# ZhengkunTian/OpenTransformer

Hardware: AMD Instinct MI355X
Metric: utterances/sec (80-d fbank, ~1000 frames) train fwd+bwd (higher is better)
Workload: dtype fp16; 1 GPU; AISHELL-1 transformer_baseline.yaml (+input_size 80), 12 enc / 6 dec layers, B=32/GPU x 1000 frames x 80-d fbank, 15 decoder rows, V=4234, residual_dropout 0.1; step = fwd + bwd + grad all-reduce + clip/Adam/Noam; global_batch=32, frames=1000, parallelism=dp1, hipgraph=True

## Files before the change

include/otrans_hip.h:

```cpp
#ifndef OTRANS_HIP_H
#define OTRANS_HIP_H
#include <stddef.h>
#include <stdint.h>
#ifdef __cplusplus
extern "C" {
#endif

#define OTR_F32 0
#define OTR_BF16 1
#define OTR_F16 2
#define OTR_ACT_NONE 0
#define OTR_ACT_RELU 1

#define OTR_ABI_VERSION 604
int32_t otr_version(void);
int32_t otr_half_type(void);
int32_t otr_debug_set(int32_t key, int32_t value);
int32_t otr_set_fault_counter(void* device_word);
int32_t otr_debug_trread(const void* image, const int32_t* addr, void* out, void* stream);
int32_t otr_debug_trace(void* buf);
const char* otr_last_error_string(void);

typedef struct {
  int32_t M, N, K;
// ... 178 lines not shown
  int32_t act_dtype, compute;
  int32_t w_dtype;
} otr_conv_desc_t;
int32_t otr_conv1_fwd(const otr_conv_desc_t* d, const float* x, const float* w1, const float* b1, void* act1,
                      void* stream);
int32_t otr_conv1_wgrad(const otr_conv_desc_t* d, const float* x, const void* dact1, float* dw1, float* db1,
                        float* partial, void* stream);
int32_t otr_conv1_wgrad_partial_rows(void);
int32_t otr_conv2_fwd(const otr_conv_desc_t* d, const void* act1, const void* w2r, const float* b2, void* act2,
                      void* stream);
int32_t otr_conv12_fwd(const otr_conv_desc_t* d, const float* x, const float* w1, const float* b1, void* act1, const void* w2r,
                       const float* b2, void* act2, void* stream);
int32_t otr_conv2_dgrad_cols(const otr_conv_desc_t* d, const void* dact2, const void* w2r, void* dcol,
                             void* stream);
int32_t otr_conv2_col2im(const otr_conv_desc_t* d, const void* dcol, const void* act1, void* dact1, void* stream);
int32_t otr_conv2_dgrad(const otr_conv_desc_t* d, const void* dact2, const void* w2r, const void* act1, void* dact1,
                        void* stream);
int64_t otr_conv2_wide_scratch_bytes(void);
int32_t otr_conv2_dgrad_wide(const otr_conv_desc_t* d, const void* dact2, const void* w2r, const void* act1, void* dact1, void* scratch,
                             int64_t scratch_bytes, void* stream);
int32_t otr_debug_conv2_dgrad_plan(const otr_conv_desc_t* d, int32_t* out);
int32_t otr_conv2_wgrad(const otr_conv_desc_t* d, const void* dact2, const void* act1, float* dw2r, void* workspace,
                        int64_t workspace_bytes, void* stream);
int32_t otr_relu_bwd(const void* y, const void* g, void* out, int32_t dtype, int64_t n, void* stream);
int32_t otr_relu_bwd_colsum_partial_rows(int64_t rows, int32_t cols, int32_t dtype);
int32_t otr_relu_bwd_colsum(const void* y, const void* g, void* out, float* partial, int32_t dtype, int64_t rows, int32_t cols,
                            void* stream);

int32_t otr_act_fwd(const void* x, void* y, int32_t dtype, int64_t n, int32_t kind, void* stream);
int32_t otr_act_bwd(const void* x, const void* dy, void* dx, int32_t dtype, int64_t n, int32_t kind, void* stream);

int32_t otr_label_smoothing_loss(const float* logits, const int64_t* target, int64_t R, int32_t V, float smoothing,
                                 int32_t pad_idx, float* loss, float* dlogits, float* scratch, void* stream);
int32_t otr_label_smoothing_loss_ld(const float* logits, int64_t ld_logits, const int64_t* target, int64_t R, int32_t V,
                                    float smoothing, int32_t pad_idx, float* loss, float* dlogits, int64_t ld_dlogits,
                                    float* scratch, void* stream);

int32_t otr_label_smoothing_loss_fused(const float* logits, int64_t ld_logits, const int64_t* target, int64_t ld_target, int32_t L,
                                       int64_t R, int32_t V, float smoothing, int32_t pad_idx, const float* grad_scale, float* loss,
                                       void* dlogits, int32_t dlogits_dtype, int64_t ld_dlogits, float* scratch, uint32_t* ticket,
                                       void* stream);

int32_t otr_log_softmax(const float* x, float* y, int64_t R, int32_t V, void* stream);

int32_t otr_residual_add_fwd(const float* x, const void* a, int32_t a_dtype, float* y, int64_t n, float scale,
                             float p_drop, const uint64_t* seed, uint64_t rng_offset, void* stream);
// ... 197 lines not shown
```

opentransformer_amd/_lib.py:

```python
import ctypes as C
import os

_HERE = os.path.dirname(os.path.abspath(__file__))
_LIB_DIR = os.environ.get('OTR_LIB_DIR') or os.path.join(_HERE, 'lib')
LIB_PATHS = {'bf16': os.path.join(_LIB_DIR, 'libotrans_hip.so'), 'fp16': os.path.join(_LIB_DIR, 'libotrans_hip_f16.so')}
LIB_PATH = LIB_PATHS['bf16']

OTR_F32, OTR_BF16, OTR_F16 = 0, 1, 2
OTR_ABI_VERSION = 604
OTR_OPT_STATE_FLOATS = 528
ACT_NONE, ACT_RELU = 0, 1


class LinearDesc(C.Structure):
    _fields_ = [('M', C.c_int32), ('N', C.c_int32), ('K', C.c_int32),
                ('x_dtype', C.c_int32), ('w_dtype', C.c_int32), ('y_dtype', C.c_int32), ('compute', C.c_int32),
                ('ldx', C.c_int64), ('ldw', C.c_int64), ('ldy', C.c_int64),
                ('act', C.c_int32), ('accumulate', C.c_int32)]


class WgradItem(C.Structure):
    _fields_ = [('dy', C.c_void_p), ('x', C.c_void_p), ('dw', C.c_void_p), ('M', C.c_int32), ('N', C.c_int32),
                ('K', C.c_int32), ('ldy', C.c_int64), ('ldx', C.c_int64), ('ldw', C.c_int64),
                ('dy_dtype', C.c_int32), ('x_dtype', C.c_int32), ('dbias', C.c_void_p), ('overwrite', C.c_int32)]
# ... 109 lines not shown
    'otr_glu_fwd': [_P, _P, _I32, _I64, _I64, _P, _P],
    'otr_glu_bwd': [_P, _P, _P, _P, _I32, _I64, _I64, _P, _I32, _P],
    'otr_posenc_fwd': [_P, _P, _P, _I64, _I32, _I32, _F32, _P],
    'otr_posenc_mask_fwd': [_P, _P, _P, _I64, _I32, _I32, _F32, _P, _I64, _I64, _P, _P],
    'otr_embed_posenc_fwd': [_P, _P, _P, _P, _I64, _I32, _I32, _I32, _F32, _P],
    'otr_embed_posenc_fwd_ld': [_P, _I64, _P, _P, _P, _I64, _I32, _I32, _I32, _F32, _P],
    'otr_embed_bwd_ld': [_P, _I64, _I32, _P, _P, _I32, _P, _I64, _I32, _I32, _F32, _P],
    'otr_embed_bwd': [_P, _P, _P, _I64, _I32, _I32, _F32, _P],
    'otr_scale': [_P, _P, _I64, _P, _F32, _P],
    'otr_scale_cast': [_P, _P, _I64, _F32, _P],
    'otr_cast_f32_to_bf16': [_P, _P, _I64, _P],
    'otr_conv1_fwd': [C.POINTER(ConvDesc), _P, _P, _P, _P, _P],
    'otr_conv1_wgrad': [C.POINTER(ConvDesc), _P, _P, _P, _P, _P, _P],
    'otr_conv1_wgrad_partial_rows': [],
    'otr_conv2_fwd': [C.POINTER(ConvDesc), _P, _P, _P, _P, _P],
    'otr_conv12_fwd': [C.POINTER(ConvDesc), _P, _P, _P, _P, _P, _P, _P, _P],
    'otr_conv2_dgrad_cols': [C.POINTER(ConvDesc), _P, _P, _P, _P],
    'otr_conv2_col2im': [C.POINTER(ConvDesc), _P, _P, _P, _P],
    'otr_conv2_dgrad': [C.POINTER(ConvDesc), _P, _P, _P, _P, _P],
    'otr_conv2_wide_scratch_bytes': [],
    'otr_conv2_dgrad_wide': [C.POINTER(ConvDesc), _P, _P, _P, _P, _P, _I64, _P],
    'otr_debug_conv2_dgrad_plan': [C.POINTER(ConvDesc), _P],
    'otr_conv2_wgrad': [C.POINTER(ConvDesc), _P, _P, _P, _P, _I64, _P],
    'otr_relu_bwd': [_P, _P, _P, _I32, _I64, _P],
    'otr_relu_bwd_colsum_partial_rows': [_I64, _I32, _I32],
    'otr_relu_bwd_colsum': [_P, _P, _P, _P, _I32, _I64, _I32, _P],
    'otr_act_fwd': [_P, _P, _I32, _I64, _I32, _P],
    'otr_act_bwd': [_P, _P, _P, _I32, _I64, _I32, _P],
    'otr_label_smoothing_loss': [_P, _P, _I64, _I32, _F32, _I32, _P, _P, _P, _P],
    'otr_label_smoothing_loss_ld': [_P, _I64, _P, _I64, _I32, _F32, _I32, _P, _P, _I64, _P, _P],
    'otr_label_smoothing_loss_fused': [_P, _I64, _P, _I64, _I32, _I64, _I32, _F32, _I32, _P, _P, _P, _I32, _I64, _P, _P, _P],
    'otr_log_softmax': [_P, _P, _I64, _I32, _P],
    'otr_ctc_loss': [_P, _P, _I64, _P, _P, _I32, _I32, _I32, _I32, _I32, _P, _P, _P, _P, _P],
    'otr_ffn_fwd_split_slab': [_P, _P, _P, _P, _P, _P, _P, _I64, _I32, _I32, _P],
    'otr_ffn_bwd_split_slab': [_P, _P, _P, _P, _P, _P, _I64, _I32, _I32, _P],
    'otr_ln_bwd_proj_slabs': [_P, _P, _I32, _P, _P, _P, _P, _P, _P, _P, _P, _P, _I64, _P, _I64, _I32, _F32, C.c_uint64, _P],
    'otr_rb_linear_ln': [C.POINTER(DecLn), _P, _P, _P, _I32, _I64, _I64, _I32, _I32, _P],
    'otr_dec_self_fwd': [C.POINTER(DecLn), _I32, _I32, _P, _P, _P, _P, _P, _P, _P, _P],
    'otr_dec_self_step': [C.POINTER(DecLn), _I64, _P, _P, _P, _P, _P, _P, _P, _I32, _P, _P],
    'otr_dec_cross_fwd': [C.POINTER(DecLn), _I32, _I32, _P, _P, _P, _P, _I64, _I64, _I32, _I32, _P, _I32, _P, _P, _P, _P, _P],
    'otr_dec_cross_fwd_shared': [C.POINTER(DecLn), _I32, _I32, _P, _P, _P, _P, _I64, _I64, _I32, _I32, _P, _I32, _I32, _P, _P, _P, _P, _P],
    'otr_dec_ffn_hsave_bytes': [_I64, _I32],
    'otr_dec_ffn_fwd': [C.POINTER(DecLn), _I64, _P, _P, _P, _I32, _I32, _P, _P, _P],
    'otr_dec_ln': [C.POINTER(DecLn), _I64, _P],
    'otr_dec_self_step_pair': [C.POINTER(DecSelfStep), C.POINTER(DecSelfStep), _P],
    'otr_dec_ffn_fwd_pair': [C.POINTER(DecFfnFwd), C.POINTER(DecFfnFwd), _P],
# ... 116 lines not shown
```

opentransformer_amd/csrc/api.hip:

```cpp
#include <stdarg.h>
#include <stdio.h>
#include <stdlib.h>

#include <algorithm>
#include <vector>

#include "gemm_kernel.h"
#include "wgrad256.h"

static thread_local char g_err[512] = "";

void otr_set_error(const char* fmt, ...) {
  va_list ap;
  va_start(ap, fmt);
  vsnprintf(g_err, sizeof(g_err), fmt, ap);
  va_end(ap);
}

int32_t otr_check_launch(const char* what) {
  hipError_t e = hipGetLastError();
  if (e != hipSuccess) {
    otr_set_error("%s: launch failed: %s", what, hipGetErrorString(e));
    return (int32_t)e;
  }
// ... 369 lines not shown
}

extern "C" int32_t otr_conv2_dgrad_cols(const otr_conv_desc_t* d, const void* dact2, const void* w2r, void* dcol,
                                        void* stream) {
  GemmArgs a{};
  if (int32_t e = conv_geom(d, a.cg)) return e;
  OTR_REQUIRE(dact2 && w2r && dcol, "conv2_dgrad_cols: null pointer");
  a.A = dact2; a.B = w2r; a.C = dcol; a.bias = nullptr;
  a.M = d->B * d->T2 * d->F2; a.N = 9 * d->C1; a.K = d->C2;
  a.lda = d->C2; a.ldb = 9 * d->C1; a.ldc = 9 * d->C1;
  a.act = OTR_ACT_NONE; a.accumulate = 0;
  a.a_vec = kc_vec(dact2, a.lda, d->act_dtype);
  OTR_REQUIRE(dtype_ok(d->w_dtype), "conv2_dgrad_cols: bad w_dtype");
  a.b_vec = mc_vec(w2r, a.ldb, d->w_dtype, d->compute);
  return run_gemm(a, d->compute, d->act_dtype, d->w_dtype, d->act_dtype, MODE_KC, MODE_MC, stream);
}

extern "C" int32_t otr_conv2_wgrad(const otr_conv_desc_t* d, const void* dact2, const void* act1, float* dw2r,
                                   void* workspace, int64_t workspace_bytes, void* stream) {
  GemmArgs a{};
  if (int32_t e = conv_geom(d, a.cg)) return e;
  OTR_REQUIRE(dact2 && act1 && dw2r, "conv2_wgrad: null pointer");
  if (g_otr_conv2_wgrad256 && d->act_dtype == OTR_H16 && d->compute == OTR_H16) {
    const int32_t rc = wgrad256_conv_launch(dact2, act1, dw2r, d->B, d->T1, d->F1, d->T2, d->F2, d->C1, d->C2, workspace, workspace_bytes,
                                            (hipStream_t)stream);
    if (rc != 1) return rc;
  }
  a.A = dact2; a.B = act1; a.C = dw2r; a.bias = nullptr;
  a.M = d->C2; a.N = 9 * d->C1; a.K = d->B * d->T2 * d->F2;
  a.lda = d->C2; a.ldb = 0; a.ldc = 9 * d->C1;
  a.act = OTR_ACT_NONE; a.accumulate = 0;
  a.a_vec = mc_vec(dact2, a.lda, d->act_dtype, d->compute);
  a.b_vec = ((uintptr_t)act1 % 16 == 0);
  a.allow_split = 1; a.ws = (float*)workspace; a.ws_bytes = workspace_bytes; a.trace = g_otr_trace;
  return run_gemm(a, d->compute, d->act_dtype, d->act_dtype, OTR_F32, MODE_MC, MODE_IM2M, stream);
}
```

opentransformer_amd/csrc/wgrad256.h:

```cpp
#pragma once
#include <hip/hip_runtime.h>
#include <stdint.h>

#include "common.h"

constexpr int W256_MAX_PROBS = 56;

struct W256Item {
  const void* dy;
  const void* x;
  float* dw;
  float* dbias;
  int M, N, K;
  int64_t ldy, ldx, ldw;
  int overwrite;
};

struct W256Prob {
  const uint16_t* dy;
  const uint16_t* x;
  float* dw;
  float* dbias;
  int start;
  int M, N, K, ldy, ldx, ldw;
  int flag0;
};

struct W256Args {
  W256Prob p[W256_MAX_PROBS];
  int total, chunk;
  int mode, nfull, rem_tiles, parts;
  int nprob, spin_limit;
  int cT1, cF1, cT2, cF2, cC1;
  FastDiv cdivF2, cdivT2;
  float* split_ws;
  int* flags;
  const void* zeros;
  int* fault;
};

int32_t wgrad256_launch(const W256Item* items, int n, void* workspace, int64_t workspace_bytes, int grid_cap, hipStream_t s);
int64_t wgrad256_workspace_bytes(const W256Item* items, int n);
int32_t wgrad256_conv_launch(const void* g2, const void* act1, float* dw2r, int B, int T1, int F1, int T2, int F2, int C1, int C2,
                             void* workspace, int64_t workspace_bytes, hipStream_t s);
```

opentransformer_amd/csrc/wgrad256.hip:

```cpp
#include "common.h"
#include "wgrad256.h"

#include <algorithm>

namespace {

typedef short v4s __attribute__((ext_vector_type(4)));
typedef __attribute__((address_space(3))) v4s lds_v4s;

constexpr int SLAB_ROWS = 16;
constexpr int SLAB_BYTES = 16384;
constexpr int RING = 8, AHEAD = 6;
constexpr int LDS_BYTES = RING * SLAB_BYTES;

__device__ __forceinline__ uint2 tr_read(uint32_t lds_addr) {
  v4s r = __builtin_amdgcn_ds_read_tr16_b64_v4i16((lds_v4s*)(uintptr_t)lds_addr);
  return __builtin_bit_cast(uint2, r);
}

struct Frags {
  uint4 a[4], b[2];
};

__device__ __forceinline__ void read_frags_lo(Frags& f, uint32_t slab_addr, uint32_t a_off, uint32_t b_off) {
// ... 24 lines not shown
#else
  typedef __bf16 hv2 __attribute__((ext_vector_type(2)));
  const hv2 one = {(__bf16)1.f, (__bf16)1.f};
#define W256_DOT(w, c) __builtin_amdgcn_fdot2_f32_bf16(__builtin_bit_cast(hv2, w), one, c, false)
#endif
#pragma unroll
  for (int a = 0; a < 4; ++a) {
    cs[a] = W256_DOT(f.a[a].x, cs[a]);
    cs[a] = W256_DOT(f.a[a].y, cs[a]);
    cs[a] = W256_DOT(f.a[a].z, cs[a]);
    cs[a] = W256_DOT(f.a[a].w, cs[a]);
  }
#undef W256_DOT
}

struct Stager {
  const unsigned char* base_a;
  const unsigned char* base_b;
  int64_t step_a, step_b;
  int row0, M;
  bool col_a, col_b;
  const unsigned char* zeros;
  uint32_t dst;
  int cT1, cF1, cT2, cF2, kh, kw;
  int64_t pix_bytes;
  FastDiv divF2, divT2;
  template <bool NTA, bool NTB, bool CONV = false> __device__ __forceinline__ void issue(int slab, int slot) {
    const bool ok = slab * SLAB_ROWS + row0 < M;
    const unsigned char* pa = ok && col_a ? base_a + slab * step_a : zeros;
    const unsigned char* pb;
    if constexpr (CONV) {
      const uint32_t m = (uint32_t)(slab * SLAB_ROWS + row0);
      const uint32_t t = fdiv(m, divF2), f2 = m - t * (uint32_t)cF2, b = fdiv(t, divT2), t2 = t - b * (uint32_t)cT2;
      const int fin = 2 * (int)f2 + kw - 1;
      const bool in = ok && col_b && fin >= 0 && fin < cF1;
      pb = in ? base_b + (((int64_t)b * cT1 + 2 * (int)t2 + kh) * cF1 + fin) * pix_bytes : zeros;
    } else {
      pb = ok && col_b ? base_b + slab * step_b : zeros;
    }
    lds_dma<NTA>(pa, (uint32_t)(slot * SLAB_BYTES) + dst);
    lds_dma<NTB>(pb, (uint32_t)(slot * SLAB_BYTES) + 8192u + dst);
  }
};

template <bool NTA, bool NTB, bool BIAS, bool CONV = false>
__device__ __forceinline__ void stream_piece(Stager& sg, f32x16 (&acc)[4][2], float (&cs)[4], int wc, int sb, int P, int rot,
                                             uint32_t a_off, uint32_t b_off) {
  int stage = rot;
  auto issue_next = [&](int slot) {
    sg.issue<NTA, NTB, CONV>(sb + stage, slot);
    stage = stage + 1 == P ? 0 : stage + 1;
  };
#pragma unroll
  for (int j = 0; j < AHEAD; ++j)
    if (j < P) issue_next(j);
  if (P >= AHEAD) wait_vm<2 * (AHEAD - 2)>(); else wait_vm<0>();
  __builtin_amdgcn_s_barrier();
  __builtin_amdgcn_sched_barrier(0);
  asm volatile("" ::: "memory");
  Frags f0, f1;
  read_frags_lo(f0, 0u, a_off, b_off);
  read_frags_hi(f0, 0u, a_off, b_off);
#define W256_MMA(A, CUR)                                                                                     \
  mma32(acc[A][0], CUR.a[A], CUR.b[0]);                                                                      \
  mma32(acc[A][1], CUR.a[A], CUR.b[1]);                                                                      \
  __builtin_amdgcn_sched_barrier(0);
#define W256_PHASE(Q, CUR, NXT, ST)                                                                          \
  {                                                                                                          \
    const int q_ = (Q);                                                                                      \
    const bool more_ = (ST) || q_ + AHEAD < P, next_ = (ST) || q_ + 1 < P;                      \
    const uint32_t nslab_ = (uint32_t)(((q_ + 1) & (RING - 1)) * SLAB_BYTES);                                \
    W256_MMA(0, CUR)                                                                                         \
    if (more_) issue_next((q_ + AHEAD) & (RING - 1));                                                        \
    __builtin_amdgcn_sched_barrier(0);                                                                       \
    W256_MMA(1, CUR)                                                                                         \
    if (next_) read_frags_lo(NXT, nslab_, a_off, b_off);                                                     \
    __builtin_amdgcn_sched_barrier(0);                                                                       \
    W256_MMA(2, CUR)                                                                                         \
    if (next_) read_frags_hi(NXT, nslab_, a_off, b_off);                                                     \
    __builtin_amdgcn_sched_barrier(0);                                                                       \
    W256_MMA(3, CUR)                                                                                         \
    if constexpr (BIAS) { if ((q_ & 3) == wc) frag_colsum(cs, CUR); }     \
    if (more_) wait_vm<2 * (AHEAD - 2)>(); else wait_vm<0>();                                                \
    __builtin_amdgcn_s_barrier();                                                                            \
    asm volatile("" ::: "memory");                                                                           \
    __builtin_amdgcn_sched_barrier(0);                                                                       \
  }
  int q = 0;
  for (; q + AHEAD + 1 < P; q += 2) {
    W256_PHASE(q, f0, f1, true)
    W256_PHASE(q + 1, f1, f0, true)
  }
  for (; q + 1 < P; q += 2) {
    W256_PHASE(q, f0, f1, false)
    W256_PHASE(q + 1, f1, f0, false)
  }
  if (q < P) W256_PHASE(q, f0, f1, false)
#undef W256_PHASE
#undef W256_MMA
}

template <bool COH, bool FIRST = false>
__device__ __forceinline__ void flush_tile(f32x16 (&acc)[4][2], float* dw, int ldw, int N, int K, int n_base, int k_base,
                                           unsigned char* scr, int lane) {
  constexpr int AUX = COH ? 17 : 0;
  const int rr = lane >> 3, cq = lane & 7;
// ... 40 lines not shown
  }
}

template <bool COH> __device__ __forceinline__ void flush_bias(const float (&cs)[4], float* dbias, int N, int n_base, int lane) {
  constexpr int AUX = COH ? 17 : 0;
  auto rs = __builtin_amdgcn_make_buffer_rsrc(dbias, 0, N * 4, 0x00020000);
#pragma unroll
  for (int a = 0; a < 4; ++a) {
    const uint32_t off = (uint32_t)((n_base + 32 * a + lane) * 4);
    const float old = __uint_as_float(__builtin_amdgcn_raw_buffer_load_b32(rs, off, 0, AUX));
    __builtin_amdgcn_raw_buffer_store_b32(__float_as_uint(old + cs[a]), rs, off, 0, AUX);
  }
}

__global__ void trread_probe_kernel(const uint16_t* image, const int* addr, uint16_t* out) {
  __shared__ __attribute__((aligned(16))) uint16_t img[2048];
  for (int i = threadIdx.x; i < 2048; i += 64) img[i] = image[i];
  __syncthreads();
  const uint2 r = tr_read((uint32_t)(uintptr_t)(lds_byte*)reinterpret_cast<unsigned char*>(img) + (uint32_t)addr[threadIdx.x]);
  out[threadIdx.x * 4 + 0] = (uint16_t)(r.x & 0xffffu); out[threadIdx.x * 4 + 1] = (uint16_t)(r.x >> 16);
  out[threadIdx.x * 4 + 2] = (uint16_t)(r.y & 0xffffu); out[threadIdx.x * 4 + 3] = (uint16_t)(r.y >> 16);
}

__global__ void wgrad256_init_kernel(int* flags, int n, uint32_t* zeros) {
  for (int i = threadIdx.x; i < n; i += blockDim.x) flags[i] = 0;
  if (threadIdx.x < 16) zeros[threadIdx.x] = 0u;
}

template <bool CONV = false>
__global__ __launch_bounds__(512) void wgrad256_kernel(W256Args g) {
  __shared__ __attribute__((aligned(1024))) unsigned char smem[LDS_BYTES];
  const int tid = threadIdx.x, lane = tid & 63;
  const int wid = __builtin_amdgcn_readfirstlane(tid >> 6);
  const int wr = wid >> 2, wc = wid & 3;
  const uint32_t smem0 = (uint32_t)(uintptr_t)(lds_byte*)smem;

  const int gq = lane >> 4, p16 = lane & 15;
  const uint32_t lane_off = (uint32_t)((4 * (gq >> 1) + (p16 >> 2)) * 64 + (gq & 1) * 32 + (p16 & 3) * 8);
  const uint32_t a_off = smem0 + lane_off + (uint32_t)(4 * wr) * 512u;
  const uint32_t b_off = smem0 + lane_off + 8192u + (uint32_t)(2 * wc) * 512u;

  const int st_row = 8 * (wid >> 2) + ((lane >> 2) & 7);
  const int st_col = 64 * (wid & 3) + 32 * (lane >> 5) + 8 * (lane & 3);

  const int G = (int)gridDim.x, gx = G >> 3, bid = (int)blockIdx.x;
  const bool rounds = g.mode >= 1;
  const int slot = (G & 7) == 0 ? (bid & 7) * gx + (rounds ? (bid >> 3) : gx - 1 - (bid >> 3)) : (rounds ? bid : G - 1 - bid);
  int pos = slot * g.chunk;
  const int c_end = pos + g.chunk < g.total ? pos + g.chunk : g.total;
  int round = 0;

  for (;;) {
    int pi = 0, tile, sb, P, rot = 0, slice = 0, nslices = 1;
    if constexpr (CONV) {
      if (round > 0 || slot >= g.rem_tiles * g.parts) break;
      ++round;
      const int R = g.chunk, part = slot / g.rem_tiles;
      tile = slot - part * g.rem_tiles;
      sb = (int)((int64_t)R * part / g.parts);
      P = (int)((int64_t)R * (part + 1) / g.parts) - sb;
      slice = part; nslices = g.parts;
    } else if (rounds) {
      const int R = g.chunk;
      int t;
      if (round < g.nfull) {
        t = round * G + slot; sb = 0; P = R;
// ... 11 lines not shown
      while (pi + 1 < g.nprob && g.p[pi + 1].start <= tpos) ++pi;
      tile = (tpos - g.p[pi].start) / R;
      if (nslices == 1) rot = (int)(((unsigned)pi * 40503u & 0xffu) * (unsigned)P >> 8);
    } else {
      if (pos >= c_end) break;
      while (pi + 1 < g.nprob && g.p[pi + 1].start <= pos) ++pi;
      const int R = (g.p[pi].M + SLAB_ROWS - 1) / SLAB_ROWS;
      const int rel = pos - g.p[pi].start;
      tile = rel / R;
      sb = rel - tile * R;
      const int tile_begin = g.p[pi].start + tile * R, tile_end = tile_begin + R;
      const int pe = tile_end < c_end ? tile_end : c_end;
      P = pe - pos;
      const int first_chunk = tile_begin / g.chunk, last_chunk = (tile_end - 1) / g.chunk;
      nslices = last_chunk - first_chunk + 1; slice = last_chunk - slot;
      pos = pe;
    }
    const W256Prob& pr = g.p[pi];
    const int tiles_k = (pr.K + 255) >> 8;
    const int tn = tile / tiles_k, tk = tile - tn * tiles_k;
    const int n0 = tn * 256, k0 = tk * 256;

    Stager sg;
    sg.M = pr.M; sg.row0 = st_row; sg.zeros = reinterpret_cast<const unsigned char*>(g.zeros);
    sg.col_a = n0 + st_col < pr.N; sg.col_b = k0 + st_col < pr.K;
    sg.base_a = reinterpret_cast<const unsigned char*>(pr.dy + (int64_t)st_row * pr.ldy + n0 + st_col);
    sg.base_b = reinterpret_cast<const unsigned char*>(pr.x + (int64_t)st_row * pr.ldx + k0 + st_col);
    sg.step_a = (int64_t)pr.ldy * SLAB_ROWS * 2; sg.step_b = (int64_t)pr.ldx * SLAB_ROWS * 2;
    sg.dst = smem0 + (uint32_t)wid * 1024u;
    if constexpr (CONV) {
      const int tap = k0 / g.cC1, ch0 = k0 - tap * g.cC1;
      sg.kh = tap / 3; sg.kw = tap - 3 * sg.kh;
      sg.cT1 = g.cT1; sg.cF1 = g.cF1; sg.cT2 = g.cT2; sg.cF2 = g.cF2; sg.divF2 = g.cdivF2; sg.divT2 = g.cdivT2;
      sg.pix_bytes = (int64_t)g.cC1 * 2;
      sg.base_b = reinterpret_cast<const unsigned char*>(pr.x + ch0 + st_col);
    }

    f32x16 acc[4][2];
#pragma unroll
    for (int a = 0; a < 4; ++a)
#pragma unroll
      for (int b = 0; b < 2; ++b)
#pragma unroll
        for (int r = 0; r < 16; ++r) acc[a][b][r] = 0.f;

    float cs[4] = {0.f, 0.f, 0.f, 0.f};
    const bool bias = pr.dbias != nullptr && tk == 0;
    const bool nt_a = tiles_k == 1, nt_b = pr.N <= 256;
#define W256_RUN(A, B)                                                                                       \
  {                                                                                                          \
    if (bias) stream_piece<A, B, true>(sg, acc, cs, wc, sb, P, rot, a_off, b_off);                     \
    else stream_piece<A, B, false>(sg, acc, cs, wc, sb, P, rot, a_off, b_off);                               \
  }
    if constexpr (CONV) stream_piece<false, false, false, true>(sg, acc, cs, wc, sb, P, rot, a_off, b_off);
    else if (nt_a && nt_b) W256_RUN(true, true)
    else if (nt_a) W256_RUN(true, false)
    else if (nt_b) W256_RUN(false, true)
    else W256_RUN(false, false)
#undef W256_RUN
    if (bias) {
      float* bx = reinterpret_cast<float*>(smem);
#pragma unroll
      for (int a = 0; a < 4; ++a) {
        cs[a] += __shfl_xor(cs[a], 32);
        if (lane < 32) bx[(wid * 4 + a) * 32 + lane] = cs[a];
      }
      __syncthreads();
      if (wc == 0 && lane < 32) {
#pragma unroll
        for (int a = 0; a < 4; ++a)
          cs[a] = bx[((wr * 4 + 0) * 4 + a) * 32 + lane] + bx[((wr * 4 + 1) * 4 + a) * 32 + lane] +
                  bx[((wr * 4 + 2) * 4 + a) * 32 + lane] + bx[((wr * 4 + 3) * 4 + a) * 32 + lane];
      }
      __syncthreads();
    }
    float* dw = pr.dw;
    const int n_base = n0 + 128 * wr, k_base = k0 + 64 * wc;
// ... 92 lines not shown
  const int64_t need = 64 + (int64_t)flags * 4;
  if (!workspace || workspace_bytes < need) {
    otr_set_error("wgrad256: workspace of %lld bytes, need %lld", (long long)workspace_bytes, (long long)need);
    return -1;
  }
  g.zeros = workspace;
  g.flags = reinterpret_cast<int*>(reinterpret_cast<unsigned char*>(workspace) + 64);
  hipLaunchKernelGGL(wgrad256_init_kernel, dim3(1), dim3(256), 0, s, g.flags, flags, reinterpret_cast<uint32_t*>(workspace));
  hipLaunchKernelGGL(wgrad256_kernel<>, dim3((unsigned)grid), dim3(512), 0, s, g);
  return otr_check_launch("wgrad256");
}

__global__ __launch_bounds__(256) void w256_reduce_kernel(const float* __restrict__ ws, int nslab, int64_t elems, float* __restrict__ dw) {
  const int64_t i = ((int64_t)blockIdx.x * 256 + threadIdx.x) * 4;
  if (i >= elems) return;
  float4 a = *reinterpret_cast<const float4*>(ws + i);
  for (int s = 1; s < nslab; ++s) {
    const float4 v = *reinterpret_cast<const float4*>(ws + (int64_t)s * elems + i);
    a.x += v.x; a.y += v.y; a.z += v.z; a.w += v.w;
  }
  *reinterpret_cast<float4*>(dw + i) = a;
}

int32_t wgrad256_conv_launch(const void* g2, const void* act1, float* dw2r, int B, int T1, int F1, int T2, int F2, int C1, int C2,
                             void* workspace, int64_t workspace_bytes, hipStream_t s) {
  const int64_t M = (int64_t)B * T2 * F2, K = 9ll * C1, elems = (int64_t)C2 * K;
  if (C1 % 256 != 0 || C2 % 8 != 0 || M < 16 * 2 * RING || M >= (1ll << 31) - 16) return 1;
  if (((uintptr_t)g2 | (uintptr_t)act1 | (uintptr_t)dw2r) % 16 != 0 || !workspace) return 1;
  const int tiles = ((C2 + 255) / 256) * (int)(K / 256);
  if (tiles > 256) return 1;
  const int64_t head = 256;
  int parts = 256 / tiles;
  const int64_t fit = (workspace_bytes - head) / (elems * 4);
  if (fit < parts) parts = (int)fit;
  const int R = (int)((M + SLAB_ROWS - 1) / SLAB_ROWS);
  if (parts > R / (2 * RING)) parts = R / (2 * RING);
  if (parts < 1) return 1;
  W256Args g{};
  W256Prob& p = g.p[0];
  p.dy = reinterpret_cast<const uint16_t*>(g2); p.x = reinterpret_cast<const uint16_t*>(act1); p.dw = dw2r; p.dbias = nullptr;
  p.M = (int)M; p.N = C2; p.K = (int)K; p.ldy = C2; p.ldx = C1; p.ldw = (int)K; p.start = 0; p.flag0 = 0;
  g.nprob = 1; g.total = tiles * R; g.chunk = R; g.mode = 2; g.nfull = 0; g.rem_tiles = tiles; g.parts = parts;
  g.spin_limit = g_otr_spin_limit; g.fault = g_otr_fault;
  g.cT1 = T1; g.cF1 = F1; g.cT2 = T2; g.cF2 = F2; g.cC1 = C1; g.cdivF2 = make_fastdiv((uint32_t)F2); g.cdivT2 = make_fastdiv((uint32_t)T2);
  g.zeros = workspace; g.flags = nullptr;
  g.split_ws = reinterpret_cast<float*>(reinterpret_cast<unsigned char*>(workspace) + head);
  hipLaunchKernelGGL(wgrad256_init_kernel, dim3(1), dim3(256), 0, s, nullptr, 0, reinterpret_cast<uint32_t*>(workspace));
  const int grid = (tiles * parts + 7) / 8 * 8;
  hipLaunchKernelGGL((wgrad256_kernel<true>), dim3((unsigned)grid), dim3(512), 0, s, g);
  if (int32_t e = otr_check_launch("wgrad256(conv)")) return e;
  hipLaunchKernelGGL(w256_reduce_kernel, dim3((unsigned)((elems / 4 + 255) / 256)), dim3(256), 0, s, g.split_ws, parts, elems, dw2r);
  return otr_check_launch("wgrad256(conv reduce)");
}

int64_t wgrad256_workspace_bytes(const W256Item* it, int n) {
  int64_t flags = 0;
  for (int i = 0; i < n; ++i) flags += w256_tiles(it[i]);
  return 64 + flags * 4;
}

extern "C" int32_t otr_debug_trread(const void* image, const int32_t* addr, void* out, void* stream) {
  OTR_REQUIRE(image && addr && out, "debug_trread: null pointer");
  hipLaunchKernelGGL(trread_probe_kernel, dim3(1), dim3(64), 0, (hipStream_t)stream, reinterpret_cast<const uint16_t*>(image), addr,
                     reinterpret_cast<uint16_t*>(out));
  return otr_check_launch("debug_trread");
}

extern "C" int32_t otr_debug_wgrad256_plan(const otr_wgrad_item_t* items, int32_t n, int32_t grid_cap, int32_t* out) {
  OTR_REQUIRE(items && out && n > 0 && n <= W256_MAX_PROBS, "debug_wgrad256_plan: bad arguments");
  W256Item it[W256_MAX_PROBS];
  for (int i = 0; i < n; ++i) it[i] = W256Item{items[i].dy, items[i].x, items[i].dw, items[i].dbias, items[i].M, items[i].N, items[i].K,
                                                items[i].ldy, items[i].ldx, items[i].ldw};
  W256Args g{};
  int grid = 0, flags = 0;
// ... 16 lines not shown
```

opentransformer_amd/ops.py:

```python
import contextlib
import ctypes as C
import gc
import math

import torch

from . import _lib as L

_state = {'compute': 'bf16', 'rng_offset': 0, 'seed': None}


@contextlib.contextmanager
def graph_capture(graph, **kw):
    gc.collect()
    was_enabled = gc.isenabled()
    gc.disable()
    _capture['serial'] += 1
    _capture['active'] = _capture['serial']
    try:
        with torch.cuda.graph(graph, **kw):
            yield graph
    finally:
        _capture['active'] = None
        if was_enabled:
# ... 2533 lines not shown

    @staticmethod
    def backward(ctx, dact2):
        x, w2r, act1, act2 = ctx.saved_tensors
        B, T, F, C1, C2, T1, F1, T2, F2 = ctx.desc_args
        adt = act2.dtype
        desc = L.ConvDesc(B, T, F, C1, C2, T1, F1, T2, F2, _code(adt), _compute_code(), _code(w2r.dtype))
        lib = L.load()
        p_drop, seed, offs = ctx.drop
        dact2 = dact2.contiguous()
        if p_drop > 0:
            gm = torch.empty_like(dact2)
            L.check(lib.otr_dropout(_p(dact2), _p(gm), _code(adt), dact2.numel(), p_drop, _p(seed), offs[1], _stream()), 'otr_dropout')
            dact2 = gm
        M2 = B * T2 * F2
        w1p, b1p, b2p = ctx.refs
        gw1, gb1, gb2 = grad_target(w1p), grad_target(b1p), grad_target(b2p)
        fused = relu_bwd_colsum_raw(act2.view(M2, C2), dact2.view(M2, C2))
        if fused is not None:
            g2, db2 = fused[0].view(dact2.shape), colsum_raw(fused[1], out=gb2)
        else:
            g2 = relu_bwd_raw(act2, dact2)
            db2 = colsum_raw(g2.view(M2, C2), out=gb2)
        dw2r = torch.empty((C2, 3, 3, C1), dtype=torch.float32, device=x.device)
        dact1 = torch.empty_like(act1)
        L.check(lib.otr_conv2_wgrad(C.byref(desc), _p(g2), _p(act1), _p(dw2r), _p(_workspace(x.device)), _WS_BYTES, _stream()),
                'otr_conv2_wgrad')
        rc = 1
        if _CONV2_IMPLICIT_DGRAD and C1 == 256 and C2 == 256:
            rc = lib.otr_conv2_dgrad_wide(C.byref(desc), _p(g2), _p(w2r), _p(act1), _p(dact1), _p(_workspace(x.device)), _WS_BYTES, _stream())
        if rc == 1:
            rc = lib.otr_conv2_dgrad(C.byref(desc), _p(g2), _p(w2r), _p(act1), _p(dact1), _stream()) if _CONV2_IMPLICIT_DGRAD else 1
        if rc == 1:
            dcol = torch.empty((M2, 9 * C1), dtype=adt, device=x.device)
            L.check(lib.otr_conv2_dgrad_cols(C.byref(desc), _p(g2), _p(w2r), _p(dcol), _stream()), 'otr_conv2_dgrad_cols')
            L.check(lib.otr_conv2_col2im(C.byref(desc), _p(dcol), _p(act1), _p(dact1), _stream()), 'otr_conv2_col2im')
        else:
            L.check(rc, 'otr_conv2_dgrad')
        if p_drop > 0:
            L.check(lib.otr_dropout(_p(dact1), _p(dact1), _code(adt), dact1.numel(), p_drop, _p(seed), offs[0], _stream()), 'otr_dropout')
        if gw1 is not None and gb1 is not None:
            dw1, db1 = gw1, gb1
        else:
            dwb = torch.zeros((C1 * 10,), dtype=torch.float32, device=x.device)
            dw1, db1 = dwb[:C1 * 9], dwb[C1 * 9:]
        nrow = lib.otr_conv1_wgrad_partial_rows()
        part = torch.empty((nrow, C1 * 10), dtype=torch.float32, device=x.device)
        L.check(lib.otr_conv1_wgrad(C.byref(desc), _p(x), _p(dact1), None, None, _p(part), _stream()), 'otr_conv1_wgrad')
        inpl = gw1 is not None and gb1 is not None
        colsum_raw(part[:, :C1 * 9], out=dw1.view(-1), defer=inpl)
        colsum_raw(part[:, C1 * 9:], out=db1, defer=inpl)
        gw2 = grad_target(ctx.w2_ref)
        if gw2 is not None and gw2.is_contiguous() and gw2.dtype == torch.float32:
            regroup_add(gw2, dw2r, C2, C1, 9, False)
            dw2 = None
        else:
            dw2 = dw2r.permute(0, 3, 1, 2)
        return (None, None if inpl else dw1.view(C1, 1, 3, 3), None if inpl else db1, dw2, None if gb2 is not None else db2, None)


def conv_subsample_with_dropout(x, w1, b1, w2, b2, p_drop):
    return ConvSubsampleFn.apply(x, w1, b1, w2, b2, float(p_drop))


def _gemm_ptr(kind, M, N, K, x, w, y, bias=None, accumulate=0):
    (xt, xo, ldx), (wt, wo, ldw), (yt, yo, ldy) = x, w, y
    d = L.LinearDesc(M, N, K, _code(xt.dtype), _code(wt.dtype), _code(yt.dtype), _compute_code(), ldx, ldw, ldy, 0,
                     accumulate)
    ws = _workspace(xt.device)
    lib = L.load()
    if kind == 'fwd':
        L.check(lib.otr_linear_fwd(C.byref(d), _p(xt, xo), _p(wt, wo), _p(bias), _p(yt, yo), _p(ws), _WS_BYTES, _stream()),
                'otr_linear_fwd')
    elif kind == 'dgrad':
        L.check(lib.otr_linear_dgrad(C.byref(d), _p(yt, yo), _p(wt, wo), _p(xt, xo), _p(ws), _WS_BYTES, _stream()),
                'otr_linear_dgrad')
# ... 762 lines not shown
```

Baseline: 7884 utterances/s.

## Fuse conv2 wgrad split-K reduce with regroup into gradient, add half-width conv tile

Adds otr_conv2_wgrad_into, which reduces the split-K partials and writes them straight into the (C2,C1,3,3) gradient with accumulate. This removes the separate dw2r buffer and the regroup_add pass. The conv stager is rewritten to track pixel offsets incrementally instead of doing a fastdiv per slab, and the zero-init kernel launch is dropped in favour of a static zero line. It also adds a 256-thread half-width tile for C2<=128 and lets C1=64/128 use the path. The risk is that the regroup reduce kernel does scalar, strided writes.

```diff
diff --git a/include/otrans_hip.h b/include/otrans_hip.h
--- a/include/otrans_hip.h
+++ b/include/otrans_hip.h
@@ -224,6 +224,8 @@
 int32_t otr_debug_conv2_dgrad_plan(const otr_conv_desc_t* d, int32_t* out);
 int32_t otr_conv2_wgrad(const otr_conv_desc_t* d, const void* dact2, const void* act1, float* dw2r, void* workspace,
                         int64_t workspace_bytes, void* stream);
+int32_t otr_conv2_wgrad_into(const otr_conv_desc_t* d, const void* dact2, const void* act1, float* gw2, int32_t accumulate,
+                             void* workspace, int64_t workspace_bytes, void* stream);
 int32_t otr_relu_bwd(const void* y, const void* g, void* out, int32_t dtype, int64_t n, void* stream);
 int32_t otr_relu_bwd_colsum_partial_rows(int64_t rows, int32_t cols, int32_t dtype);
 int32_t otr_relu_bwd_colsum(const void* y, const void* g, void* out, float* partial, int32_t dtype, int64_t rows, int32_t cols,
diff --git a/opentransformer_amd/_lib.py b/opentransformer_amd/_lib.py
--- a/opentransformer_amd/_lib.py
+++ b/opentransformer_amd/_lib.py
@@ -155,6 +155,7 @@
     'otr_conv2_dgrad_wide': [C.POINTER(ConvDesc), _P, _P, _P, _P, _P, _I64, _P],
     'otr_debug_conv2_dgrad_plan': [C.POINTER(ConvDesc), _P],
     'otr_conv2_wgrad': [C.POINTER(ConvDesc), _P, _P, _P, _P, _I64, _P],
+    'otr_conv2_wgrad_into': [C.POINTER(ConvDesc), _P, _P, _P, _I32, _P, _I64, _P],
     'otr_relu_bwd': [_P, _P, _P, _I32, _I64, _P],
     'otr_relu_bwd_colsum_partial_rows': [_I64, _I32, _I32],
     'otr_relu_bwd_colsum': [_P, _P, _P, _P, _I32, _I64, _I32, _P],
diff --git a/opentransformer_amd/csrc/api.hip b/opentransformer_amd/csrc/api.hip
--- a/opentransformer_amd/csrc/api.hip
+++ b/opentransformer_amd/csrc/api.hip
@@ -415,8 +415,8 @@
   if (int32_t e = conv_geom(d, a.cg)) return e;
   OTR_REQUIRE(dact2 && act1 && dw2r, "conv2_wgrad: null pointer");
   if (g_otr_conv2_wgrad256 && d->act_dtype == OTR_H16 && d->compute == OTR_H16) {
-    const int32_t rc = wgrad256_conv_launch(dact2, act1, dw2r, d->B, d->T1, d->F1, d->T2, d->F2, d->C1, d->C2, workspace, workspace_bytes,
-                                            (hipStream_t)stream);
+    const int32_t rc = wgrad256_conv_launch(dact2, act1, dw2r, nullptr, 0, d->B, d->T1, d->F1, d->T2, d->F2, d->C1, d->C2, workspace,
+                                            workspace_bytes, (hipStream_t)stream);
     if (rc != 1) return rc;
   }
   a.A = dact2; a.B = act1; a.C = dw2r; a.bias = nullptr;
@@ -428,3 +428,13 @@
   a.allow_split = 1; a.ws = (float*)workspace; a.ws_bytes = workspace_bytes; a.trace = g_otr_trace;
   return run_gemm(a, d->compute, d->act_dtype, d->act_dtype, OTR_F32, MODE_MC, MODE_IM2M, stream);
 }
+
+extern "C" int32_t otr_conv2_wgrad_into(const otr_conv_desc_t* d, const void* dact2, const void* act1, float* gw2, int32_t accumulate,
+                                        void* workspace, int64_t workspace_bytes, void* stream) {
+  ConvGeom cg{};
+  if (int32_t e = conv_geom(d, cg)) return e;
+  OTR_REQUIRE(dact2 && act1 && gw2, "conv2_wgrad_into: null pointer");
+  if (!(g_otr_conv2_wgrad256 && d->act_dtype == OTR_H16 && d->compute == OTR_H16)) return 1;
+  return wgrad256_conv_launch(dact2, act1, nullptr, gw2, accumulate, d->B, d->T1, d->F1, d->T2, d->F2, d->C1, d->C2, workspace,
+                              workspace_bytes, (hipStream_t)stream);
+}
diff --git a/opentransformer_amd/csrc/wgrad256.h b/opentransformer_amd/csrc/wgrad256.h
--- a/opentransformer_amd/csrc/wgrad256.h
+++ b/opentransformer_amd/csrc/wgrad256.h
@@ -41,5 +41,5 @@
 
 int32_t wgrad256_launch(const W256Item* items, int n, void* workspace, int64_t workspace_bytes, int grid_cap, hipStream_t s);
 int64_t wgrad256_workspace_bytes(const W256Item* items, int n);
-int32_t wgrad256_conv_launch(const void* g2, const void* act1, float* dw2r, int B, int T1, int F1, int T2, int F2, int C1, int C2,
-                             void* workspace, int64_t workspace_bytes, hipStream_t s);
+int32_t wgrad256_conv_launch(const void* g2, const void* act1, float* dw2r, float* grad, int accumulate, int B, int T1, int F1, int T2,
+                             int F2, int C1, int C2, void* workspace, int64_t workspace_bytes, hipStream_t s);
diff --git a/opentransformer_amd/csrc/wgrad256.hip b/opentransformer_amd/csrc/wgrad256.hip
--- a/opentransformer_amd/csrc/wgrad256.hip
+++ b/opentransformer_amd/csrc/wgrad256.hip
@@ -70,39 +70,69 @@
   bool col_a, col_b;
   const unsigned char* zeros;
   uint32_t dst;
-  int cT1, cF1, cT2, cF2, kh, kw;
-  int64_t pix_bytes;
-  FastDiv divF2, divT2;
-  template <bool NTA, bool NTB, bool CONV = false> __device__ __forceinline__ void issue(int slab, int slot) {
+  template <bool NTA, bool NTB, bool HALF = false> __device__ __forceinline__ void issue(int slab, int slot) {
     const bool ok = slab * SLAB_ROWS + row0 < M;
     const unsigned char* pa = ok && col_a ? base_a + slab * step_a : zeros;
-    const unsigned char* pb;
-    if constexpr (CONV) {
-      const uint32_t m = (uint32_t)(slab * SLAB_ROWS + row0);
-      const uint32_t t = fdiv(m, divF2), f2 = m - t * (uint32_t)cF2, b = fdiv(t, divT2), t2 = t - b * (uint32_t)cT2;
-      const int fin = 2 * (int)f2 + kw - 1;
-      const bool in = ok && col_b && fin >= 0 && fin < cF1;
-      pb = in ? base_b + (((int64_t)b * cT1 + 2 * (int)t2 + kh) * cF1 + fin) * pix_bytes : zeros;
-    } else {
-      pb = ok && col_b ? base_b + slab * step_b : zeros;
-    }
+    const unsigned char* pb = ok && col_b ? base_b + slab * step_b : zeros;
     lds_dma<NTA>(pa, (uint32_t)(slot * SLAB_BYTES) + dst);
     lds_dma<NTB>(pb, (uint32_t)(slot * SLAB_BYTES) + 8192u + dst);
   }
 };
 
-template <bool NTA, bool NTB, bool BIAS, bool CONV = false>
-__device__ __forceinline__ void stream_piece(Stager& sg, f32x16 (&acc)[4][2], float (&cs)[4], int wc, int sb, int P, int rot,
+struct ConvStager {
+  const unsigned char* cur_a;
+  const unsigned char* base_b;
+  const unsigned char* zeros;
+  int64_t step_a;
+  int row0, M;
+  bool col_a;
+  uint32_t dst, dst_b;
+  uint32_t pix_bytes;
+  uint32_t pixel;
+  int f2, t2, cF2, cT2;
+  uint32_t row_step, batch_step;
+  int64_t tap_off[2];
+  int f_lo[2], f_hi[2];
+  __device__ __forceinline__ void start(int slab, const uint16_t* dy, int ldy, int col, int T1, int F1) {
+    const uint32_t m = (uint32_t)(slab * SLAB_ROWS + row0);
+    const uint32_t t = m / (uint32_t)cF2, b = t / (uint32_t)cT2;
+    f2 = (int)(m - t * (uint32_t)cF2); t2 = (int)(t - b * (uint32_t)cT2);
+    pixel = (b * (uint32_t)T1 + 2u * (uint32_t)t2) * (uint32_t)F1 + 2u * (uint32_t)f2;
+    row_step = 2u * (uint32_t)(F1 - cF2); batch_step = (uint32_t)(T1 - 2 * cT2) * (uint32_t)F1;
+    cur_a = reinterpret_cast<const unsigned char*>(dy + (int64_t)m * ldy + col);
+    step_a = (int64_t)ldy * SLAB_ROWS * 2;
+  }
+  template <bool NTA, bool NTB, bool HALF> __device__ __forceinline__ void issue(int slab, int slot) {
+    const bool ok = slab * SLAB_ROWS + row0 < M;
+    lds_dma<false>(ok && col_a ? cur_a : zeros, (uint32_t)(slot * SLAB_BYTES) + dst);
+    const unsigned char* pix = base_b + (uint64_t)pixel * pix_bytes;
+#pragma unroll
+    for (int j = 0; j < (HALF ? 2 : 1); ++j) {
+      const bool in = ok && f2 >= f_lo[j] && f2 <= f_hi[j];
+      lds_dma<false>(in ? pix + tap_off[j] : zeros, (uint32_t)(slot * SLAB_BYTES) + dst_b + (uint32_t)j * 1024u);
+    }
+    cur_a += step_a;
+    f2 += SLAB_ROWS; pixel += 2u * SLAB_ROWS;
+    while (f2 >= cF2) {
+      f2 -= cF2; pixel += row_step;
+      if (++t2 == cT2) { t2 = 0; pixel += batch_step; }
+    }
+  }
+};
+
+template <bool NTA, bool NTB, bool BIAS, bool HALF = false, class SG>
+__device__ __forceinline__ void stream_piece(SG& sg, f32x16 (&acc)[4][2], float (&cs)[4], int wc, int sb, int P, int rot,
                                              uint32_t a_off, uint32_t b_off) {
+  constexpr int INFLIGHT = (HALF ? 3 : 2) * (AHEAD - 2);
   int stage = rot;
   auto issue_next = [&](int slot) {
-    sg.issue<NTA, NTB, CONV>(sb + stage, slot);
+    sg.template issue<NTA, NTB, HALF>(sb + stage, slot);
     stage = stage + 1 == P ? 0 : stage + 1;
   };
 #pragma unroll
   for (int j = 0; j < AHEAD; ++j)
     if (j < P) issue_next(j);
-  if (P >= AHEAD) wait_vm<2 * (AHEAD - 2)>(); else wait_vm<0>();
+  if (P >= AHEAD) wait_vm<INFLIGHT>(); else wait_vm<0>();
   __builtin_amdgcn_s_barrier();
   __builtin_amdgcn_sched_barrier(0);
   asm volatile("" ::: "memory");
@@ -129,7 +159,7 @@
     __builtin_amdgcn_sched_barrier(0);                                                                       \
     W256_MMA(3, CUR)                                                                                         \
     if constexpr (BIAS) { if ((q_ & 3) == wc) frag_colsum(cs, CUR); }     \
-    if (more_) wait_vm<2 * (AHEAD - 2)>(); else wait_vm<0>();                                                \
+    if (more_) wait_vm<INFLIGHT>(); else wait_vm<0>();                                                         \
     __builtin_amdgcn_s_barrier();                                                                            \
     asm volatile("" ::: "memory");                                                                           \
     __builtin_amdgcn_sched_barrier(0);                                                                       \
@@ -216,17 +246,20 @@
   out[threadIdx.x * 4 + 2] = (uint16_t)(r.y & 0xffffu); out[threadIdx.x * 4 + 3] = (uint16_t)(r.y >> 16);
 }
 
+__device__ const uint4 w256_zero_line[4] = {};
+
 __global__ void wgrad256_init_kernel(int* flags, int n, uint32_t* zeros) {
   for (int i = threadIdx.x; i < n; i += blockDim.x) flags[i] = 0;
   if (threadIdx.x < 16) zeros[threadIdx.x] = 0u;
 }
 
-template <bool CONV = false>
-__global__ __launch_bounds__(512) void wgrad256_kernel(W256Args g) {
+template <bool CONV = false, bool HALF = false>
+__global__ __launch_bounds__(HALF ? 256 : 512) void wgrad256_kernel(W256Args g) {
+  static_assert(CONV || !HALF, "the half-width tile serves the conv form only");
   __shared__ __attribute__((aligned(1024))) unsigned char smem[LDS_BYTES];
   const int tid = threadIdx.x, lane = tid & 63;
   const int wid = __builtin_amdgcn_readfirstlane(tid >> 6);
-  const int wr = wid >> 2, wc = wid & 3;
+  const int wr = HALF ? 0 : wid >> 2, wc = wid & 3;
   const uint32_t smem0 = (uint32_t)(uintptr_t)(lds_byte*)smem;
 
   const int gq = lane >> 4, p16 = lane & 15;
@@ -234,8 +267,10 @@
   const uint32_t a_off = smem0 + lane_off + (uint32_t)(4 * wr) * 512u;
   const uint32_t b_off = smem0 + lane_off + 8192u + (uint32_t)(2 * wc) * 512u;
 
-  const int st_row = 8 * (wid >> 2) + ((lane >> 2) & 7);
-  const int st_col = 64 * (wid & 3) + 32 * (lane >> 5) + 8 * (lane & 3);
+  const int st_row = HALF ? 8 * (wid >> 1) + ((lane >> 2) & 7) : 8 * (wid >> 2) + ((lane >> 2) & 7);
+  const int st_lc = 32 * (lane >> 5) + 8 * (lane & 3);
+  const int st_col_a = (HALF ? 64 * (wid & 1) : 64 * (wid & 3)) + st_lc;
+  const int st_col = (HALF ? 128 * (wid & 1) : 64 * (wid & 3)) + st_lc;
 
   const int G = (int)gridDim.x, gx = G >> 3, bid = (int)blockIdx.x;
   const bool rounds = g.mode >= 1;
@@ -293,18 +328,32 @@
     const int n0 = tn * 256, k0 = tk * 256;
 
     Stager sg;
-    sg.M = pr.M; sg.row0 = st_row; sg.zeros = reinterpret_cast<const unsigned char*>(g.zeros);
-    sg.col_a = n0 + st_col < pr.N; sg.col_b = k0 + st_col < pr.K;
-    sg.base_a = reinterpret_cast<const unsigned char*>(pr.dy + (int64_t)st_row * pr.ldy + n0 + st_col);
-    sg.base_b = reinterpret_cast<const unsigned char*>(pr.x + (int64_t)st_row * pr.ldx + k0 + st_col);
-    sg.step_a = (int64_t)pr.ldy * SLAB_ROWS * 2; sg.step_b = (int64_t)pr.ldx * SLAB_ROWS * 2;
-    sg.dst = smem0 + (uint32_t)wid * 1024u;
+    ConvStager cg;
     if constexpr (CONV) {
-      const int tap = k0 / g.cC1, ch0 = k0 - tap * g.cC1;
-      sg.kh = tap / 3; sg.kw = tap - 3 * sg.kh;
-      sg.cT1 = g.cT1; sg.cF1 = g.cF1; sg.cT2 = g.cT2; sg.cF2 = g.cF2; sg.divF2 = g.cdivF2; sg.divT2 = g.cdivT2;
-      sg.pix_bytes = (int64_t)g.cC1 * 2;
-      sg.base_b = reinterpret_cast<const unsigned char*>(pr.x + ch0 + st_col);
+      cg.M = pr.M; cg.row0 = st_row; cg.zeros = reinterpret_cast<const unsigned char*>(w256_zero_line);
+      cg.col_a = n0 + st_col_a < pr.N;
+      cg.dst = smem0 + (HALF ? (uint32_t)(wid >> 1) * 4096u + (uint32_t)(wid & 1) * 1024u : (uint32_t)wid * 1024u);
+      cg.dst_b = smem0 + 8192u + (HALF ? (uint32_t)(wid >> 1) * 4096u + (uint32_t)(wid & 1) * 2048u : (uint32_t)wid * 1024u);
+      cg.cT2 = g.cT2; cg.cF2 = g.cF2;
+      cg.pix_bytes = (uint32_t)g.cC1 * 2u;
+      cg.base_b = reinterpret_cast<const unsigned char*>(pr.x);
+#pragma unroll
+      for (int j = 0; j < (HALF ? 2 : 1); ++j) {
+        const int kk = k0 + st_col + 64 * j;
+        const int tap = kk / g.cC1, ch = kk - tap * g.cC1, kh = tap / 3, kw = tap - 3 * kh;
+        const bool has_tap = kk < pr.K;
+        cg.tap_off[j] = ((int64_t)(kh * g.cF1 + kw - 1) * g.cC1 + ch) * 2;
+        cg.f_lo[j] = has_tap ? (kw == 0 ? 1 : 0) : 1;
+        cg.f_hi[j] = has_tap ? min(g.cF2 - 1, (g.cF1 - kw) >> 1) : 0;
+      }
+      cg.start(sb, pr.dy, pr.ldy, n0 + st_col_a, g.cT1, g.cF1);
+    } else {
+      sg.M = pr.M; sg.row0 = st_row; sg.zeros = reinterpret_cast<const unsigned char*>(g.zeros);
+      sg.col_a = n0 + st_col < pr.N; sg.col_b = k0 + st_col < pr.K;
+      sg.base_a = reinterpret_cast<const unsigned char*>(pr.dy + (int64_t)st_row * pr.ldy + n0 + st_col);
+      sg.base_b = reinterpret_cast<const unsigned char*>(pr.x + (int64_t)st_row * pr.ldx + k0 + st_col);
+      sg.step_a = (int64_t)pr.ldy * SLAB_ROWS * 2; sg.step_b = (int64_t)pr.ldx * SLAB_ROWS * 2;
+      sg.dst = smem0 + (uint32_t)wid * 1024u;
     }
 
     f32x16 acc[4][2];
@@ -323,7 +372,7 @@
     if (bias) stream_piece<A, B, true>(sg, acc, cs, wc, sb, P, rot, a_off, b_off);                     \
     else stream_piece<A, B, false>(sg, acc, cs, wc, sb, P, rot, a_off, b_off);                               \
   }
-    if constexpr (CONV) stream_piece<false, false, false, true>(sg, acc, cs, wc, sb, P, rot, a_off, b_off);
+    if constexpr (CONV) stream_piece<false, false, false, HALF>(cg, acc, cs, wc, sb, P, rot, a_off, b_off);
     else if (nt_a && nt_b) W256_RUN(true, true)
     else if (nt_a) W256_RUN(true, false)
     else if (nt_b) W256_RUN(false, true)
@@ -462,12 +511,28 @@
   *reinterpret_cast<float4*>(dw + i) = a;
 }
 
-int32_t wgrad256_conv_launch(const void* g2, const void* act1, float* dw2r, int B, int T1, int F1, int T2, int F2, int C1, int C2,
-                             void* workspace, int64_t workspace_bytes, hipStream_t s) {
+__global__ __launch_bounds__(256) void w256_reduce_regroup_kernel(const float* __restrict__ ws, int nslab, int64_t elems, int C1,
+                                                                  float* __restrict__ grad, int accumulate) {
+  const int64_t i = (int64_t)blockIdx.x * 256 + threadIdx.x;
+  if (i >= elems) return;
+  float a = ws[i];
+#pragma unroll 8
+  for (int s = 1; s < nslab; ++s) a += ws[(int64_t)s * elems + i];
+  const int K = 9 * C1;
+  const int n = (int)(i / K), k = (int)(i - (int64_t)n * K), tap = k / C1, c = k - tap * C1;
+  float* d = grad + ((int64_t)n * C1 + c) * 9 + tap;
+  *d = accumulate ? *d + a : a;
+}
+
+int32_t wgrad256_conv_launch(const void* g2, const void* act1, float* dw2r, float* grad, int accumulate, int B, int T1, int F1, int T2,
+                             int F2, int C1, int C2, void* workspace, int64_t workspace_bytes, hipStream_t s) {
   const int64_t M = (int64_t)B * T2 * F2, K = 9ll * C1, elems = (int64_t)C2 * K;
-  if (C1 % 256 != 0 || C2 % 8 != 0 || M < 16 * 2 * RING || M >= (1ll << 31) - 16) return 1;
-  if (((uintptr_t)g2 | (uintptr_t)act1 | (uintptr_t)dw2r) % 16 != 0 || !workspace) return 1;
-  const int tiles = ((C2 + 255) / 256) * (int)(K / 256);
+  if ((C1 != 64 && C1 != 128 && C1 % 256 != 0) || C2 % 8 != 0 || M < 16 * 2 * RING || M >= (1ll << 31) - 16) return 1;
+  if ((int64_t)B * T1 * F1 >= (1ll << 31)) return 1;
+  float* out = grad ? grad : dw2r;
+  if (((uintptr_t)g2 | (uintptr_t)act1 | (uintptr_t)out) % 16 != 0 || !out || !workspace) return 1;
+  const bool half = C2 <= 128;
+  const int tiles = ((C2 + 255) / 256) * (int)((K + 255) / 256);
   if (tiles > 256) return 1;
   const int64_t head = 256;
   int parts = 256 / tiles;
@@ -483,13 +548,17 @@
   g.nprob = 1; g.total = tiles * R; g.chunk = R; g.mode = 2; g.nfull = 0; g.rem_tiles = tiles; g.parts = parts;
   g.spin_limit = g_otr_spin_limit; g.fault = g_otr_fault;
   g.cT1 = T1; g.cF1 = F1; g.cT2 = T2; g.cF2 = F2; g.cC1 = C1; g.cdivF2 = make_fastdiv((uint32_t)F2); g.cdivT2 = make_fastdiv((uint32_t)T2);
-  g.zeros = workspace; g.flags = nullptr;
+  g.zeros = nullptr; g.flags = nullptr;
   g.split_ws = reinterpret_cast<float*>(reinterpret_cast<unsigned char*>(workspace) + head);
-  hipLaunchKernelGGL(wgrad256_init_kernel, dim3(1), dim3(256), 0, s, nullptr, 0, reinterpret_cast<uint32_t*>(workspace));
   const int grid = (tiles * parts + 7) / 8 * 8;
-  hipLaunchKernelGGL((wgrad256_kernel<true>), dim3((unsigned)grid), dim3(512), 0, s, g);
+  if (half) hipLaunchKernelGGL((wgrad256_kernel<true, true>), dim3((unsigned)grid), dim3(256), 0, s, g);
+  else hipLaunchKernelGGL((wgrad256_kernel<true>), dim3((unsigned)grid), dim3(512), 0, s, g);
   if (int32_t e = otr_check_launch("wgrad256(conv)")) return e;
-  hipLaunchKernelGGL(w256_reduce_kernel, dim3((unsigned)((elems / 4 + 255) / 256)), dim3(256), 0, s, g.split_ws, parts, elems, dw2r);
+  if (grad)
+    hipLaunchKernelGGL(w256_reduce_regroup_kernel, dim3((unsigned)((elems + 255) / 256)), dim3(256), 0, s, g.split_ws, parts, elems, C1, grad,
+                       accumulate);
+  else
+    hipLaunchKernelGGL(w256_reduce_kernel, dim3((unsigned)((elems / 4 + 255) / 256)), dim3(256), 0, s, g.split_ws, parts, elems, dw2r);
   return otr_check_launch("wgrad256(conv reduce)");
 }
 
diff --git a/opentransformer_amd/ops.py b/opentransformer_amd/ops.py
--- a/opentransformer_amd/ops.py
+++ b/opentransformer_amd/ops.py
@@ -2579,10 +2579,16 @@
         else:
             g2 = relu_bwd_raw(act2, dact2)
             db2 = colsum_raw(g2.view(M2, C2), out=gb2)
-        dw2r = torch.empty((C2, 3, 3, C1), dtype=torch.float32, device=x.device)
+        gw2 = grad_target(ctx.w2_ref)
+        gw2_direct = gw2 is not None and gw2.is_contiguous() and gw2.dtype == torch.float32
         dact1 = torch.empty_like(act1)
-        L.check(lib.otr_conv2_wgrad(C.byref(desc), _p(g2), _p(act1), _p(dw2r), _p(_workspace(x.device)), _WS_BYTES, _stream()),
-                'otr_conv2_wgrad')
+        dw2r, rc = None, 1
+        if gw2_direct:
+            rc = lib.otr_conv2_wgrad_into(C.byref(desc), _p(g2), _p(act1), _p(gw2), 1, _p(_workspace(x.device)), _WS_BYTES, _stream())
+        if rc == 1:
+            dw2r = torch.empty((C2, 3, 3, C1), dtype=torch.float32, device=x.device)
+            rc = lib.otr_conv2_wgrad(C.byref(desc), _p(g2), _p(act1), _p(dw2r), _p(_workspace(x.device)), _WS_BYTES, _stream())
+        L.check(rc, 'otr_conv2_wgrad')
         rc = 1
         if _CONV2_IMPLICIT_DGRAD and C1 == 256 and C2 == 256:
             rc = lib.otr_conv2_dgrad_wide(C.byref(desc), _p(g2), _p(w2r), _p(act1), _p(dact1), _p(_workspace(x.device)), _WS_BYTES, _stream())
@@ -2607,8 +2613,9 @@
         inpl = gw1 is not None and gb1 is not None
         colsum_raw(part[:, :C1 * 9], out=dw1.view(-1), defer=inpl)
         colsum_raw(part[:, C1 * 9:], out=db1, defer=inpl)
-        gw2 = grad_target(ctx.w2_ref)
-        if gw2 is not None and gw2.is_contiguous() and gw2.dtype == torch.float32:
+        if dw2r is None:
+            dw2 = None
+        elif gw2_direct:
             regroup_add(gw2, dw2r, C2, C1, 9, False)
             dw2 = None
         else:
```

Result: no change. 7936 utterances/s, median of 6 (+0.7%).
